# rkhosrowshahi/MO-VAE

Hardware: AMD Instinct MI355X
Metric: training images/sec (higher is better)
Workload: dtype f32

## Files before the change

### mo-vae_amd/csrc/conv_igemm.hip

```cpp
#include <cstring>
#include <cstdio>
#include "common.h"
#include <stdlib.h>

namespace {

constexpr int BK = 16;

struct Geom {
    int Nimg;
    int Hi, Wi, Cr;
    int Ho, Wo, Nn;
    int KH, KW, stride, pad;
    int wrow, wlen, wstride, woff;
};

struct Epilogue {
    const float* bias;
    int act;
    float slope;
};

struct ActMul {
    const float* y;
// ... 834 lines not shown
    RSide none{};
    if (!g_defer.pending || g_defer.st != st || g_bench_main_only) return none;
    if (g_defer.bytes > (pair ? defer_max_bytes_pair() : defer_max_bytes())) {
        (void)defer_flush();
        return none;
    }
    g_defer.pending = false;
    ++g_defer_stats[1];
    return g_defer.r;
}

inline RSide defer_take_3d(hipStream_t st, dim3* g, int* gz) {
    *gz = (int)g->z;
    RSide none{};
    if (!g_defer.pending || g_defer.st != st || g_bench_main_only) return none;
    const long layers = ((long)g_defer.r.nblk + (long)g->x * g->y - 1) / ((long)g->x * g->y);
    if ((long)g->z + layers > 65535) return none;
    if (g_defer.bytes > defer_max_bytes()) {
        (void)defer_flush();
        return none;
    }
    g->z += (unsigned)layers;
    return defer_take(st, false);
}

inline int launch_reduce_groups(const float* slab, const RGroups& rg, int G, long n1, long n2, int S, int N, const float* bias, int act,
                                float slope, int accumulate, hipStream_t st, ActMul am = ActMul{nullptr, 0, 0.f, 0, 0, nullptr},
                                bool deferrable = false) {
    if (g_bench_main_only) return MOVAE_OK;
    const long total = n1 + n2;
    uintptr_t al = reinterpret_cast<uintptr_t>(slab) | (uintptr_t)(rg.slab_gs * 4);
    for (int i = 0; i < G; ++i) al |= reinterpret_cast<uintptr_t>(rg.out[i]) | reinterpret_cast<uintptr_t>(rg.out2[i]);
    const bool al16 = (al & 15) == 0;
    RSide r{slab, rg, total, n1, S, N, accumulate, 0, 0, 0};
    if (S >= 64 && total % 4 == 0 && n1 % 4 == 0 && total <= (1L << 20) && al16) {
        r.kind = 0, r.nbx = (int)ceil_div(total, 16);
    } else if (S >= 8 && total >= reduce_vec_min() && total % 4 == 0 && n1 % 4 == 0 && al16) {
        r.kind = 1, r.nbx = (int)ceil_div(total / 4, 256);
    } else if (S >= 8 && total <= (1L << 20)) {
        r.kind = 2, r.nbx = (int)ceil_div(total, 16);
    } else {
        long gq = (total + 255) / 256;
        if (gq > 4096) gq = 4096;
        r.kind = 3, r.nbx = (int)gq;
    }
    r.nblk = r.nbx * G;
    static const char* const kind_name[4] = {"splitk_reduce_wide", "splitk_reduce_vec", "splitk_reduce", "splitk_reduce_flat"};
    note_reduce(kind_name[r.kind]);
    if (deferrable && g_defer.armed && !bias && act == MOVAE_ACT_NONE && !am.y && !am.res &&
        (size_t)total * S * G * sizeof(float) <= (defer_max_bytes() > defer_max_bytes_pair() ? defer_max_bytes() : defer_max_bytes_pair())) {
        if (int rc = defer_flush()) return rc;
        g_defer.r = r, g_defer.st = st, g_defer.pending = true, g_defer.bytes = (size_t)total * S * G * sizeof(float);
        ++g_defer.serial;
        ++g_defer_stats[0];
        return MOVAE_OK;
    }
    return reduce_launch(r, bias, act, slope, am, st);
}

inline int launch_reduce(const float* slab, float* out, long n1, int S, int N, const float* bias, int act, float slope,
                         int accumulate, hipStream_t st, float* out2 = nullptr, long n2 = 0, ActMul am = ActMul{nullptr, 0, 0.f, 0, 0, nullptr}) {
    if (!out2) n2 = 0;
    RGroups rg{};
    rg.out[0] = out, rg.out2[0] = out2, rg.slab_gs = 0;
    return launch_reduce_groups(slab, rg, 1, n1, n2, S, N, bias, act, slope, accumulate, st, am);
}

inline bool reduce_stats_shape_ok(const void* slab, const void* out, const void* part, const void* bias, long M, int N) {
    return N % 4 == 0 && N <= 1024 && 256 % (N / 4) == 0 && M <= 0x7fffffffL &&
           ((reinterpret_cast<uintptr_t>(slab) | reinterpret_cast<uintptr_t>(out) | reinterpret_cast<uintptr_t>(part)) & 15) == 0 &&
           (!bias || (reinterpret_cast<uintptr_t>(bias) & 15) == 0);
}

inline bool launch_reduce_stats(const float* slab, float* out, long M, int N, int S, const ClsSplit* scls, int Ho, int Wo, int stride,
                                const float* bias, hipStream_t st) {
    if (!g_fuse.stats || !reduce_stats_shape_ok(slab, out, g_fuse.stats, bias, M, N)) return false;
    const int RG = 256 / (N / 4);
    long rpb = 2L * RG;
    if ((M + rpb - 1) / rpb > 1024) rpb = ((M + 1023) / 1024 + RG - 1) / RG * RG;
    const long nblk = (M + rpb - 1) / rpb;
    float* part = fuse_stats_claim(nblk, N);
    if (!part) return false;
    ClsSplit one{{S, S, S, S}};
    note_reduce("splitk_reduce_stats");
    hipLaunchKernelGGL(splitk_reduce_stats, dim3((unsigned)nblk), dim3(256), 0, st, slab, out, (int)M, N, S, scls ? *scls : one, Ho, Wo,
                       scls ? stride : 0, bias, part, (int)rpb, BnBwd{});
    return true;
}

inline bool plan_reduce_bnbwd(long M, int N, BnBwd* bb, int* rows_per_block) {
    if (!g_fuse.bn_y || !g_fuse.bn_part || N % 4 != 0 || N > 1024 || 256 % (N / 4) != 0 || M > 0x7fffffffL || M % g_fuse.bn_groups != 0)
        return false;
    const long rpg = M / g_fuse.bn_groups;
    const int RG = 256 / (N / 4);
    long rpb = 2L * RG;
    while (rpb > RG && rpg % rpb != 0) rpb -= RG;
    if (rpg % rpb != 0) return false;
    while (rpg / rpb * g_fuse.bn_groups > 2048 && rpg % (rpb * 2) == 0) rpb *= 2;
    float* part = fuse_bn_claim(rpg / rpb, N);
    if (!part || ((reinterpret_cast<uintptr_t>(part) | reinterpret_cast<uintptr_t>(g_fuse.bn_y) | reinterpret_cast<uintptr_t>(g_fuse.bn_scale) |
                   reinterpret_cast<uintptr_t>(g_fuse.bn_shift)) & 15) != 0) {
        g_fuse.bn_ppg = 0;
        return false;
    }
    *bb = BnBwd{g_fuse.bn_y, g_fuse.bn_scale, g_fuse.bn_shift, g_fuse.bn_slope, part, (int)rpg, (int)(rpg / rpb)};
    *rows_per_block = (int)rpb;
    return true;
}

inline void launch_reduce_bnbwd(const float* slab, float* out, long M, int N, int S, const ClsSplit* scls, int Ho, int Wo, int stride,
                                const BnBwd& bb, int rows_per_block, hipStream_t st) {
    ClsSplit one{{S, S, S, S}};
    note_reduce("splitk_reduce_stats");
    hipLaunchKernelGGL(splitk_reduce_stats, dim3((unsigned)((M + rows_per_block - 1) / rows_per_block)), dim3(256), 0, st, slab, out, (int)M,
                       N, S, scls ? *scls : one, Ho, Wo, scls ? stride : 0, (const float*)nullptr, (float*)nullptr, rows_per_block, bb);
}

enum { FORM_FWD = 0, FORM_BWD = 1, FORM_WGRAD = 2 };
inline int choose_split(int form, int tile_area, int bk, long tiles, int nk, size_t per_slab_bytes, size_t ws_bytes, bool have_ws) {
    if (!have_ws || nk < 2) return 1;
    long smax = nk < 256 ? nk : 256;
    while (smax > 1 && per_slab_bytes * (size_t)smax > ws_bytes) --smax;
    if (g_force_split > 0) return (int)(g_force_split < smax ? g_force_split : smax);
    const bool big = tile_area >= 128 * 128;
    const double form_tk = form == FORM_FWD ? 1.0 : (form == FORM_BWD ? 1.25 : 0.9);
    const double tk = form_tk * (tile_area / 4096.0) * (big ? 0.83 : 1.0) * (bk / 32.0);
    const double out_mb = (double)per_slab_bytes * 1e-6;
    int best = 1;
    double best_t = 0.0;
    for (long S = 1; S <= smax; ++S) {
        const long kps = (nk + S - 1) / S;
        if ((nk + kps - 1) / kps != S) continue;
        const long blocks = tiles * S;
        const long rounds = (blocks + 511) / 512;
        const double share = blocks <= 256 ? 1.0 : 1.6;
        double t = rounds * (2.0 + kps * tk * share);
        if (S > 1) t += 2.5 + S * out_mb * 0.87;
        if (S == 1 || t < best_t * 0.97) {
            best = (int)S;
            best_t = t;
        }
    }
    return best;
}

inline bool pair_collecting();
template <class Plan>
inline void pair_stash(const Plan& p);
inline int pair_flush(hipStream_t st);
#include "igemm_v2.h"
#include "conv_thin.h"
#include "linear_small.h"
#include "kgemm.h"
#include "pair.h"
namespace kg {
inline bool g_force_kgemm_on() { return g_force_kgemm > 0; }
}

inline bool is_linear(const Geom& g) {
    return g.KH == 1 && g.KW == 1 && g.Hi == 1 && g.Wi == 1 && g.Ho == 1 && g.Wo == 1 && g.stride == 1 && g.pad == 0 && g.wlen == 0;
}

inline bool aligned16(const void* p) { return (reinterpret_cast<uintptr_t>(p) & 15) == 0; }

inline long big_tile_min() {
    static const long v = env_long("MOVAE_BIG_TILE_MIN", 256);
    return g_big_tile_min > 0 ? g_big_tile_min : v;
}

template <int BM, int BN>
int launch_fwd_t(const float* X, const float* W, float* Y, const Geom& g, const Epilogue& ep, int M, int K, bool vec,
                 void* ws, size_t ws_bytes, hipStream_t st) {
    const int gx = ceil_div(M, BM), gy = ceil_div(g.Nn, BN);
    const int nk = ceil_div(K, BK);
    const long tiles = (long)gx * gy;
    int S = choose_split(FORM_FWD, BM * BN, BK, tiles, nk, (size_t)M * g.Nn * sizeof(float), ws_bytes, ws != nullptr);
    const int per_split = ceil_div(nk, S);
    S = ceil_div(nk, per_split);
    float* slab = S > 1 ? static_cast<float*>(ws) : nullptr;
    dim3 grid(gx, gy, S);
    if (vec)
        hipLaunchKernelGGL((igemm_fwd<BM, BN, true>), grid, dim3(256), 0, st, X, W, Y, g, ep, M, K, per_split, slab);
    else
        hipLaunchKernelGGL((igemm_fwd<BM, BN, false>), grid, dim3(256), 0, st, X, W, Y, g, ep, M, K, per_split, slab);
    MOVAE_CHECK_LAUNCH("igemm_fwd");
    if (S > 1) {
        const long total = (long)M * g.Nn;
        if (int rc = launch_reduce(slab, Y, total, S, g.Nn, ep.bias, ep.act, ep.slope, 0, st)) return rc;
    }
    return MOVAE_OK;
}

inline bool tap_window(const Geom& g, Geom* out) {
    static const bool enabled = !getenv("MOVAE_NO_TAPWIN");
    if (!enabled || g.Ho != 1 || g.Wo != 1 || g.pad >= g.KH || g.pad >= g.KW) return false;
    const int nkh = g.KH - g.pad < g.Hi ? g.KH - g.pad : g.Hi, nkw = g.KW - g.pad < g.Wi ? g.KW - g.pad : g.Wi;
    if (nkh < 1 || nkw < 1 || nkh * nkw == g.KH * g.KW) return false;
    *out = g;
    out->KH = nkh, out->KW = nkw, out->pad = 0;
    out->wrow = g.KH * g.KW * g.Cr;
    out->wlen = nkw * g.Cr, out->wstride = g.KW * g.Cr, out->woff = (g.pad * g.KW + g.pad) * g.Cr;
    return true;
}

int launch_fwd(const float* X, const float* W, float* Y, const Geom& g_in, const Epilogue& ep, void* ws, size_t ws_bytes,
               hipStream_t st) {
    Geom g = g_in;
    {
        const long Kfull = (long)g.KH * g.KW * g.Cr;
        Geom gw;
        if (g.Cr % 4 == 0 && aligned16(X) && aligned16(W) && !is_linear(g) && !thin::thin_in_ok(g) && g.Nn > 4 && Kfull <= 0x7fffffffL &&
            tap_window(g, &gw))
            g = gw;
    }
    const long Ml = (long)g.Nimg * g.Ho * g.Wo;
    const long Kl = (long)g.KH * g.KW * g.Cr;
    if (Ml <= 0 || g.Nn <= 0 || Kl <= 0 || Ml > 0x7fffffffL) {
        movae_set_error("conv fwd-form: bad shape M=%ld N=%d K=%ld", Ml, g.Nn, Kl);
        return MOVAE_EINVAL;
    }
    const int M = (int)Ml, K = (int)Kl;
    if (is_linear(g) && lin::linear_small_ok(Ml, g.Nn, Kl) && aligned16(X) && aligned16(W)) {
        MOVAE_NO_NORM("linear (fwd)");
        float* ys[1] = {Y};
        return (g_last_kernel = "linear_small_k<NT>",
                lin::launch_linear_small<0>(X, W, ys, nullptr, 1, 0, ep.bias, M, g.Nn, K, ep.act, ep.slope, 0, st));
    }
    if (thin::thin_in_ok(g)) {
        MOVAE_NO_NORM("thin-channel input conv");
        return thin::launch_thin_in<false>(X, W, Y, g, ep, st);
    }
    if (g.Nn <= 4) {
        bool handled = false;
        if (int rc = thin::launch_thin_out_tile<false>(X, W, Y, g, ep, st, &handled)) return rc;
        if (handled) return MOVAE_OK;
    }
    if (thin::thin_out_ok(g, X)) {
        MOVAE_NO_NORM("thin-channel output conv");
        return thin::launch_thin_out_fwd(X, W, Y, g, ep, st);
    }
    const bool span_ok = v2::buf_span_ok((128L / ((long)g.Ho * g.Wo) + 2) * g.Hi * g.Wi * g.Cr) &&
                         v2::buf_span_ok((long)g.Nn * (g.wlen ? g.wrow : Kl) + g.woff);
    if (g_force_kgemm >= 0) {
        bool handled = false;
        if (int rc = kg::launch_kfwd(X, W, Y, g, ep, M, K, st, &handled)) return rc;
        if (handled) return MOVAE_OK;
    }
    if (g.Cr % 4 == 0 && aligned16(X) && aligned16(W) && span_ok) {
        if (g.Nn <= 32) return (g_last_kernel = "igemm2_fwd<128,32>", v2::launch_fwd2<128, 32>(X, W, Y, g, ep, M, K, ws, ws_bytes, st));
        if (g.Nn >= 128 && (Ml / 128) * (g.Nn / 128) >= big_tile_min()) return (g_last_kernel = g_movae_compute_bf16 ? "igemm2_fwd<128,128,true>" : "igemm2_fwd<128,128>", v2::launch_fwd2<128, 128>(X, W, Y, g, ep, M, K, ws, ws_bytes, st));
        if (Ml >= 128 * 512) return (g_last_kernel = "igemm2_fwd<128,64>", v2::launch_fwd2<128, 64>(X, W, Y, g, ep, M, K, ws, ws_bytes, st));
        return (g_last_kernel = "igemm2_fwd<64,64>", v2::launch_fwd2<64, 64>(X, W, Y, g, ep, M, K, ws, ws_bytes, st));
    }
    MOVAE_NO_NORM("generic conv (fwd form)");
    const bool vec = (g.Cr % BK == 0) && aligned16(X) && aligned16(W);
    if (g.Nn <= 32) return (g_last_kernel = vec ? "igemm_fwd<128,32,true>" : "igemm_fwd<128,32,false>", launch_fwd_t<128, 32>(X, W, Y, g, ep, M, K, vec, ws, ws_bytes, st));
    if (Ml >= 128 * 512) return (g_last_kernel = vec ? "igemm_fwd<128,64,true>" : "igemm_fwd<128,64,false>", launch_fwd_t<128, 64>(X, W, Y, g, ep, M, K, vec, ws, ws_bytes, st));
    return (g_last_kernel = vec ? "igemm_fwd<64,64,true>" : "igemm_fwd<64,64,false>", launch_fwd_t<64, 64>(X, W, Y, g, ep, M, K, vec, ws, ws_bytes, st));
}

template <int BM, int BN>
int launch_bwd_t(const float* X, const float* W, float* Y, const Geom& g, const Epilogue& ep, bool vec, void* ws,
                 size_t ws_bytes, hipStream_t st) {
    const int s = g.stride;
    const long Mmax = (long)g.Nimg * ceil_div(g.Ho, s) * ceil_div(g.Wo, s);
    const int gx = ceil_div(Mmax, BM), gy = ceil_div(g.Nn, BN);
    const int nk_max = ceil_div((long)ceil_div(g.KH, s) * ceil_div(g.KW, s) * g.Cr, BK);
    const long total = (long)g.Nimg * g.Ho * g.Wo * g.Nn;
    int S = choose_split(FORM_BWD, BM * BN, BK, (long)gx * gy * s * s, nk_max, (size_t)total * sizeof(float), ws_bytes, ws != nullptr);
    const int per_split = ceil_div(nk_max, S);
    S = ceil_div(nk_max, per_split);
    float* slab = S > 1 ? static_cast<float*>(ws) : nullptr;
    dim3 grid(gx, gy, s * s * S);
    if (vec)
        hipLaunchKernelGGL((igemm_bwd<BM, BN, true>), grid, dim3(256), 0, st, X, W, Y, g, ep, S, per_split, slab, total);
    else
        hipLaunchKernelGGL((igemm_bwd<BM, BN, false>), grid, dim3(256), 0, st, X, W, Y, g, ep, S, per_split, slab, total);
    MOVAE_CHECK_LAUNCH("igemm_bwd");
    if (S > 1) {
        if (int rc = launch_reduce(slab, Y, total, S, g.Nn, ep.bias, ep.act, ep.slope, 0, st)) return rc;
    }
    return MOVAE_OK;
}

int launch_bwd(const float* X, const float* W, float* Y, const Geom& g, const Epilogue& ep, void* ws, size_t ws_bytes,
               hipStream_t st) {
    const long Ml = (long)g.Nimg * g.Ho * g.Wo;
    if (Ml <= 0 || g.Nn <= 0 || g.Cr <= 0 || Ml > 0x7fffffffL) {
        movae_set_error("conv bwd-form: bad shape M=%ld N=%d Cr=%d", Ml, g.Nn, g.Cr);
        return MOVAE_EINVAL;
    }
    const long Mc = Ml / (g.stride * g.stride);
    if (is_linear(g) && lin::linear_small_ok(Ml, g.Nn, g.Cr) && g.Nn % 4 == 0 && aligned16(X) && aligned16(W)) {
        MOVAE_NO_NORM("linear (bwd form)");
        float* ys[1] = {Y};
        if (g_stash.collect) {
            g_stash.put(lin::make_prob<1>(X, nullptr, W, nullptr, ys, nullptr, 1, 1, 0, ep.bias, nullptr, (int)Ml, g.Nn, g.Cr, ep.act, ep.slope, 0));
            g_last_kernel = "linear_small_k<NN>";
            return MOVAE_OK;
        }
        return (g_last_kernel = "linear_small_k<NN>",
                lin::launch_linear_small<1>(X, W, ys, nullptr, 1, 0, ep.bias, (int)Ml, g.Nn, g.Cr, ep.act, ep.slope, 0, st));
    }
    if (thin::thin_in_ok(g)) {
        MOVAE_NO_NORM("thin-channel input (bwd form)");
        return thin::launch_thin_in<true>(X, W, Y, g, ep, st);
    }
    if (g.Nn <= 4) {
        bool handled = false;
        if (int rc = thin::launch_thin_out_tile<true>(X, W, Y, g, ep, st, &handled)) return rc;
        if (handled) return MOVAE_OK;
    }
    const long hwc_min = (long)(g.Ho / g.stride > 0 ? g.Ho / g.stride : 1) * (g.Wo / g.stride > 0 ? g.Wo / g.stride : 1);
    const bool span_ok = v2::buf_span_ok((128L / hwc_min + 2) * g.Hi * g.Wi * g.Cr) && v2::buf_span_ok((long)g.Cr * g.KH * g.KW * g.Nn);
    if (g_force_kgemm >= 0) {
        bool handled = false;
        if (int rc = kg::launch_kbwd(X, W, Y, g, ep, st, &handled)) return rc;
        if (handled) return MOVAE_OK;
    }
    if (g.Cr % 4 == 0 && g.Nn % 4 == 0 && g.stride <= 2 && aligned16(X) && aligned16(W) && aligned16(Y) && span_ok) {
        if (g.Nn <= 32) return (g_last_kernel = "igemm2_bwd<128,32>", v2::launch_bwd2<128, 32>(X, W, Y, g, ep, ws, ws_bytes, st));
        if (g.Nn >= 128 && (Mc / 128) * (g.Nn / 128) * g.stride * g.stride >= big_tile_min())
            return (g_last_kernel = g_movae_compute_bf16 ? "igemm2_bwd<128,128,true>" : "igemm2_bwd<128,128>", v2::launch_bwd2<128, 128>(X, W, Y, g, ep, ws, ws_bytes, st));
        if (Mc >= 128 * 512) return (g_last_kernel = "igemm2_bwd<128,64>", v2::launch_bwd2<128, 64>(X, W, Y, g, ep, ws, ws_bytes, st));
        return (g_last_kernel = "igemm2_bwd<64,64>", v2::launch_bwd2<64, 64>(X, W, Y, g, ep, ws, ws_bytes, st));
    }
    MOVAE_NO_NORM("generic conv (bwd form)");
    const bool vec = (g.Cr % BK == 0) && (g.Nn % 4 == 0) && aligned16(X) && aligned16(W);
    if (g.Nn <= 32) return (g_last_kernel = vec ? "igemm_bwd<128,32,true>" : "igemm_bwd<128,32,false>", launch_bwd_t<128, 32>(X, W, Y, g, ep, vec, ws, ws_bytes, st));
    if (Mc >= 128 * 512) return (g_last_kernel = vec ? "igemm_bwd<128,64,true>" : "igemm_bwd<128,64,false>", launch_bwd_t<128, 64>(X, W, Y, g, ep, vec, ws, ws_bytes, st));
    return (g_last_kernel = vec ? "igemm_bwd<64,64,true>" : "igemm_bwd<64,64,false>", launch_bwd_t<64, 64>(X, W, Y, g, ep, vec, ws, ws_bytes, st));
}

template <int BM, int BN>
int launch_wgrad_t(const float* S, const float* Bg, float* dW, const WGeom& g, int K, int vec, int accumulate, void* ws,
                   size_t ws_bytes, hipStream_t st) {
    const int M = g.Cs, N = g.KH * g.KW * g.Cb;
    const int gx = ceil_div(M, BM), gy = ceil_div(N, BN);
    const long tiles = (long)gx * gy;
    int Sp = choose_split(FORM_WGRAD, BM * BN, BK, tiles, ceil_div(K, BK), (size_t)M * N * sizeof(float), ws_bytes, ws != nullptr);
    int kchunk = ceil_div(ceil_div(K, Sp), BK) * BK;
    Sp = ceil_div(K, kchunk);
    const bool slab = Sp > 1 || accumulate;
    if (slab && (!ws || (size_t)M * N * sizeof(float) * Sp > ws_bytes)) {
        movae_set_error("wgrad: workspace too small (%zu bytes) for %d splits of %dx%d", ws_bytes, Sp, M, N);
        return MOVAE_EINVAL;
    }
    float* out = slab ? static_cast<float*>(ws) : dW;
    dim3 grid(gx, gy, Sp);
    const bool va = (vec & 1) != 0, vb = (vec & 2) != 0;
    if (va && vb)
        hipLaunchKernelGGL((igemm_wgrad<BM, BN, true, true>), grid, dim3(256), 0, st, S, Bg, out, g, K, kchunk, slab ? 1 : 0);
    else if (va)
        hipLaunchKernelGGL((igemm_wgrad<BM, BN, true, false>), grid, dim3(256), 0, st, S, Bg, out, g, K, kchunk, slab ? 1 : 0);
    else if (vb)
        hipLaunchKernelGGL((igemm_wgrad<BM, BN, false, true>), grid, dim3(256), 0, st, S, Bg, out, g, K, kchunk, slab ? 1 : 0);
    else
        hipLaunchKernelGGL((igemm_wgrad<BM, BN, false, false>), grid, dim3(256), 0, st, S, Bg, out, g, K, kchunk, slab ? 1 : 0);
    MOVAE_CHECK_LAUNCH("igemm_wgrad");
    if (slab) {
        const long total = (long)M * N;
        if (int rc = launch_reduce(out, dW, total, Sp, N, nullptr, 0, 0.f, accumulate, st)) return rc;
    }
    return MOVAE_OK;
}

int launch_wgrad1(const float* S, const float* Bg, float* dW, const WGeom& g, int accumulate, void* ws, size_t ws_bytes,
                  hipStream_t st) {
    const long Kl = (long)g.Nimg * g.Hs * g.Ws;
    const int vec = ((g.Cs % 4 == 0 && aligned16(S)) ? 1 : 0) | ((g.Cb % 4 == 0 && aligned16(Bg)) ? 2 : 0);
    const int N = g.KH * g.KW * g.Cb;
    if (thin::thin_wgrad_ok(g) && ws) return thin::launch_thin_wgrad(S, Bg, dW, g, (int)Kl, accumulate, ws, ws_bytes, st);
    static const char* const wgrad_name[2][4] = {
        {"igemm_wgrad<128,32,false,false>", "igemm_wgrad<128,32,true,false>", "igemm_wgrad<128,32,false,true>", "igemm_wgrad<128,32,true,true>"},
        {"igemm_wgrad<64,64,false,false>", "igemm_wgrad<64,64,true,false>", "igemm_wgrad<64,64,false,true>", "igemm_wgrad<64,64,true,true>"}};
    if (N <= 32) return (g_last_kernel = wgrad_name[0][vec], launch_wgrad_t<128, 32>(S, Bg, dW, g, (int)Kl, vec, accumulate, ws, ws_bytes, st));
    return (g_last_kernel = wgrad_name[1][vec], launch_wgrad_t<64, 64>(S, Bg, dW, g, (int)Kl, vec, accumulate, ws, ws_bytes, st));
}

int launch_wgrad(const float* S, const float* Bg, float* const* dW, int G, long s_gs, long b_gs, const WGeom& g, int accumulate,
                 void* ws, size_t ws_bytes, hipStream_t st, float* const* colsum_S = nullptr, bool* colsum_done = nullptr) {
    const long Kl = (long)g.Nimg * g.Hs * g.Ws;
    if (Kl <= 0 || Kl > 0x7fffffffL || g.Cs <= 0 || g.Cb <= 0) {
        movae_set_error("wgrad: bad shape K=%ld Cs=%d Cb=%d", Kl, g.Cs, g.Cb);
        return MOVAE_EINVAL;
    }
    if (colsum_done) *colsum_done = false;
    if (g.KH == 1 && g.KW == 1 && g.Hs == 1 && g.Ws == 1 && g.Hb == 1 && g.Wb == 1 && b_gs == 0 &&
        lin::linear_small_ok(g.Cs, g.Cb, (Kl + 3) / 4 * 4) && !g_bench_main_only) {
        MOVAE_NO_NORM("linear (wgrad)");
        if (colsum_done) *colsum_done = colsum_S != nullptr;
        if (g_stash.kind == PairStash::LINEAR) {
            g_stash.kind = PairStash::NONE, g_stash.paired = true;
            const lin::LinProb wp = lin::make_prob<2>(S, nullptr, Bg, nullptr, dW, colsum_S, G, 1, s_gs, nullptr, nullptr, g.Cs, g.Cb, (int)Kl, 0,
                                                      0.f, accumulate);
            g_last_kernel = "linear_bwd_k<false>";
            return lin::launch_linear_bwd<false>(g_stash.lin, wp, st);
        }
        return (g_last_kernel = "linear_small_k<TN>",
                lin::launch_linear_small<2>(S, Bg, dW, colsum_S, G, s_gs, nullptr, g.Cs, g.Cb, (int)Kl, 0, 0.f, accumulate, st));
    }
    const bool vec = g.Cs % 4 == 0 && g.Cb % 4 == 0 && aligned16(S) && aligned16(Bg) && s_gs % 4 == 0 && b_gs % 4 == 0 &&
                     v2::buf_span_ok(Kl * g.Cs) && v2::buf_span_ok((long)g.Nimg * g.Hb * g.Wb * g.Cb);
    const int N = g.KH * g.KW * g.Cb;
    if (g_force_kgemm >= 0 && !colsum_S && !thin::thin_wgrad_ok(g)) {
        bool handled = false;
        if (int rc = kg::launch_kwgrad(S, Bg, dW, G, s_gs, b_gs, g, (int)Kl, accumulate, ws, ws_bytes, st, &handled)) return rc;
        if (handled) return MOVAE_OK;
    }
    if (vec && !(thin::thin_wgrad_ok(g) && ws)) {
        float* const* cs = nullptr;
        if (colsum_S && !(g_fuse.nrm.scale && g_fuse.nrm_side == 1)) {
            cs = colsum_S;
            for (int i = 0; i < G; ++i)
                if (!colsum_S[i]) cs = nullptr;
        }
        if (colsum_done) *colsum_done = cs != nullptr;
        if (N <= 32) return (g_last_kernel = "igemm2_wgrad<128,32>", launch_wgrad2<128, 32>(S, Bg, dW, G, s_gs, b_gs, g, (int)Kl, accumulate, ws, ws_bytes, st, cs));
        if (g.Cs <= 32 && N >= 128) return (g_last_kernel = "igemm2_wgrad<32,128>", launch_wgrad2<32, 128>(S, Bg, dW, G, s_gs, b_gs, g, (int)Kl, accumulate, ws, ws_bytes, st, cs));
        if (g.Cs >= 128 && (long)(g.Cs / 128) * (N / 128) * (Kl / 512) * G >= big_tile_min())
            return (g_last_kernel = g_movae_compute_bf16 ? "igemm2_wgrad<128,128,true>" : "igemm2_wgrad<128,128>", launch_wgrad2<128, 128>(S, Bg, dW, G, s_gs, b_gs, g, (int)Kl, accumulate, ws, ws_bytes, st, cs));
        static const bool wide64 = !getenv("MOVAE_NO_WGRAD_64x128");
        if (wide64 && g.Cs > 32 && g.Cs <= 64 && N >= 256 && (long)(N / 128) * (Kl / 512) * G >= big_tile_min())
            return (g_last_kernel = "igemm2_wgrad<64,128>", launch_wgrad2<64, 128>(S, Bg, dW, G, s_gs, b_gs, g, (int)Kl, accumulate, ws, ws_bytes, st, cs));
        return (g_last_kernel = "igemm2_wgrad<64,64>", launch_wgrad2<64, 64>(S, Bg, dW, G, s_gs, b_gs, g, (int)Kl, accumulate, ws, ws_bytes, st, cs));
    }
    if (thin::thin_wgrad_ok(g) && ws)
        return thin::launch_thin_wgrad_grouped(S, Bg, dW, G, s_gs, b_gs, g, (int)Kl, accumulate, ws, ws_bytes, st, colsum_S, colsum_done);
    MOVAE_NO_NORM("generic wgrad");
    for (int i = 0; i < G; ++i)
        if (int rc = launch_wgrad1(S + i * s_gs, Bg + i * b_gs, dW[i], g, accumulate, ws, ws_bytes, st)) return rc;
    return MOVAE_OK;
}

int check_conv_shape(const char* who, int n, int hi, int wi, int ci, int ho, int wo, int co, int kh, int kw, int stride,
                     int pad, bool transposed) {
    if (n <= 0 || hi <= 0 || wi <= 0 || ci <= 0 || ho <= 0 || wo <= 0 || co <= 0 || kh <= 0 || kw <= 0 || stride <= 0 ||
        pad < 0) {
        movae_set_error("%s: non-positive dimension", who);
        return MOVAE_EINVAL;
    }
    if (!transposed) {
        if ((hi + 2 * pad - kh) / stride + 1 != ho || (wi + 2 * pad - kw) / stride + 1 != wo) {
            movae_set_error("%s: output %dx%d inconsistent with input %dx%d k%dx%d s%d p%d", who, ho, wo, hi, wi, kh, kw,
                            stride, pad);
            return MOVAE_EINVAL;
        }
    } else {
        const int op_h = ho - ((hi - 1) * stride - 2 * pad + kh), op_w = wo - ((wi - 1) * stride - 2 * pad + kw);
        if (op_h < 0 || op_h >= stride || op_w < 0 || op_w >= stride) {
            movae_set_error("%s: transposed output %dx%d inconsistent with input %dx%d k%dx%d s%d p%d", who, ho, wo, hi, wi,
                            kh, kw, stride, pad);
            return MOVAE_EINVAL;
        }
    }
    return MOVAE_OK;
}

}

int g_movae_compute_bf16 = 0;

struct FuseScope {
    movae_fuse_t* f;
    bool fwd;
    explicit FuseScope(movae_fuse_t* fuse, int nrm_side) : f(fuse), fwd(nrm_side == 0) {
        g_fuse = FuseCtx();
        if (!f) return;
        f->stats_parts = 0;
        if (f->in_scale && f->in_shift) g_fuse.nrm = Norm{f->in_scale, f->in_shift, f->in_slope}, g_fuse.nrm_side = nrm_side;
        if (f->stats && f->stats_cap > 0) g_fuse.stats = f->stats, g_fuse.stats_cap = f->stats_cap;
        if (fwd) {
            f->ep_act_done = 0;
            if (f->ep_res && (reinterpret_cast<uintptr_t>(f->ep_res) & 15) == 0)
                g_fuse.am = ActMul{nullptr, 0, 0.f, 0, 0, f->ep_res}, g_fuse.am_groups = 1;
        }
    }
    ~FuseScope() {
        if (f) f->stats_parts = g_fuse.stats_parts;
        if (f && fwd) f->ep_act_done = g_fuse.am_done ? 1 : 0;
        g_fuse = FuseCtx();
    }
};

struct DgradFuseScope {
    movae_fuse_t* f;
    DgradFuseScope(movae_fuse_t* fuse, int groups) : f(fuse) {
        g_fuse = FuseCtx();
        if (!f) return;
        f->bn_ppg = 0;
        f->ep_act_done = 0;
        const bool want_act = f->ep_act_y && f->ep_act != MOVAE_ACT_NONE;
        if ((want_act || f->ep_res) && groups >= 1 &&
            ((reinterpret_cast<uintptr_t>(f->ep_act_y) | reinterpret_cast<uintptr_t>(f->ep_res)) & 15) == 0)
            g_fuse.am = ActMul{want_act ? f->ep_act_y : nullptr, f->ep_act, f->ep_slope, 0, 0, f->ep_res}, g_fuse.am_groups = groups,
            g_fuse.am_done = false;
        if (f->bn_y && f->bn_scale && f->bn_shift && f->bn_part && f->bn_cap > 0 && groups >= 1) {
            g_fuse.bn_y = f->bn_y, g_fuse.bn_scale = f->bn_scale, g_fuse.bn_shift = f->bn_shift, g_fuse.bn_slope = f->bn_slope;
            g_fuse.bn_part = f->bn_part, g_fuse.bn_cap = f->bn_cap, g_fuse.bn_groups = groups;
        }
    }
    ~DgradFuseScope() {
        if (f) f->bn_ppg = g_fuse.bn_ppg, f->ep_act_done = g_fuse.am_done ? 1 : 0;
        g_fuse.bn_y = nullptr, g_fuse.bn_part = nullptr, g_fuse.bn_ppg = 0, g_fuse.bn_groups = 1;
        g_fuse.am.y = nullptr, g_fuse.am.res = nullptr, g_fuse.am_groups = 1, g_fuse.am_done = false;
    }
};
#define MOVAE_CHECK_FUSE(f, c)                                                                                                   \
    MOVAE_CHECK_ARG(!(f) || !(f)->in_scale ||                                                                                    \
                        ((f)->in_shift && (c) % 4 == 0 && ((reinterpret_cast<uintptr_t>((f)->in_scale) | reinterpret_cast<uintptr_t>((f)->in_shift)) & 15) == 0), \
                    "fused input transform: needs scale AND shift, 16-byte aligned, channels %% 4 == 0")

static int conv_fwd(bool transposed, const float* x, const float* w, const float* bias, float* y, int n, int hi, int wi, int ci, int ho,
                    int wo, int co, int kh, int kw, int stride, int pad, int act, float slope, void* ws, size_t ws_bytes,
                    movae_stream_t stream, movae_fuse_t* fuse) {
    const char* who = transposed ? "movae_convT2d_fwd" : "movae_conv2d_fwd";
    MOVAE_WS_SCRATCH(ws, ws_bytes);
    MOVAE_CHECK_ARG(x && w && y, "%s: null pointer", who);
    if (int rc = check_conv_shape(who, n, hi, wi, ci, ho, wo, co, kh, kw, stride, pad, transposed)) return rc;
    MOVAE_CHECK_FUSE(fuse, ci);
    FuseScope scope(fuse, 0);
    Geom g{n, hi, wi, ci, ho, wo, co, kh, kw, stride, pad};
    return transposed ? launch_bwd(x, w, y, g, Epilogue{bias, act, slope}, ws, ws_bytes, (hipStream_t)stream)
                      : launch_fwd(x, w, y, g, Epilogue{bias, act, slope}, ws, ws_bytes, (hipStream_t)stream);
}

static int conv_dgrad(bool transposed, const float* dy, const float* w, float* dx, int n, int hi, int wi, int ci, int ho, int wo, int co,
                      int kh, int kw, int stride, int pad, void* ws, size_t ws_bytes, movae_stream_t stream, movae_fuse_t* fuse, int groups) {
    const char* who = transposed ? "movae_convT2d_dgrad" : "movae_conv2d_dgrad";
    DgradFuseScope scope(fuse, groups);
    MOVAE_WS_SCRATCH(ws, ws_bytes);
    MOVAE_CHECK_ARG(dy && w && dx, "%s: null pointer", who);
    if (int rc = check_conv_shape(who, n, hi, wi, ci, ho, wo, co, kh, kw, stride, pad, transposed)) return rc;
    Geom g{n, ho, wo, co, hi, wi, ci, kh, kw, stride, pad};
    return transposed ? launch_fwd(dy, w, dx, g, Epilogue{nullptr, MOVAE_ACT_NONE, 0.f}, ws, ws_bytes, (hipStream_t)stream)
                      : launch_bwd(dy, w, dx, g, Epilogue{nullptr, MOVAE_ACT_NONE, 0.f}, ws, ws_bytes, (hipStream_t)stream);
}

static int conv_wgrad_grouped(bool transposed, int groups, const float* dy, const float* x, float* const* dw, float* const* dbias, int n,
                              int hi, int wi, int ci, int ho, int wo, int co, int kh, int kw, int stride, int pad, int accumulate, void* ws,
                              size_t ws_bytes, movae_stream_t stream, const movae_fuse_t* fuse) {
    const char* who = transposed ? "movae_convT2d_wgrad" : "movae_conv2d_wgrad";
    DeferArmScope defer_scope;
    MOVAE_CHECK_FUSE(fuse, ci);
    FuseScope scope(const_cast<movae_fuse_t*>(fuse), transposed ? 1 : 2);
    void* ws_full = ws;
    const size_t ws_full_bytes = ws_bytes;
    MOVAE_WS_SCRATCH(ws, ws_bytes);
    MOVAE_CHECK_ARG(dy && x && dw && groups >= 1 && groups <= 8, "%s: null pointer / bad group count", who);
    for (int i = 0; i < groups; ++i) MOVAE_CHECK_ARG(dw[i], "%s: null dw", who);
    if (int rc = check_conv_shape(who, n, hi, wi, ci, ho, wo, co, kh, kw, stride, pad, transposed)) return rc;
    const long dy_gs = (long)n * ho * wo * co;
    bool bias_done = false;
    const int rc = transposed ? launch_wgrad(x, dy, dw, groups, 0, dy_gs, WGeom{n, hi, wi, ci, ho, wo, co, kh, kw, stride, pad}, accumulate, ws,
                                             ws_bytes, (hipStream_t)stream)
                              : launch_wgrad(dy, x, dw, groups, dy_gs, 0, WGeom{n, ho, wo, co, hi, wi, ci, kh, kw, stride, pad}, accumulate, ws,
                                             ws_bytes, (hipStream_t)stream, dbias, &bias_done);
    if (rc) return rc;
    if (dbias && !bias_done && !g_bench_main_only && g_defer.pending && g_defer.serial != defer_scope.serial)
        if (int rc2 = defer_flush()) return rc2;
    if (dbias && !bias_done && !g_bench_main_only)
        for (int i = 0; i < groups; ++i)
            if (dbias[i])
                if (int rc2 = movae_colsum(dy + i * dy_gs, dbias[i], n * ho * wo, co, accumulate, ws_full, ws_full_bytes, stream)) return rc2;
    return MOVAE_OK;
}

static int conv_dgrad_wgrad_grouped(bool transposed, int groups, const float* dy, const float* w, const float* x, float* dx, float* const* dw,
                                    float* const* dbias, int n, int hi, int wi, int ci, int ho, int wo, int co, int kh, int kw, int stride,
                                    int pad, int accumulate, void* ws, size_t ws_bytes, movae_stream_t stream, const movae_fuse_t* fuse) {
    static const bool enabled = !getenv("MOVAE_NO_PAIR");
    MOVAE_CHECK_ARG(dx && w, "%s: null pointer", transposed ? "movae_convT2d_dgrad_wgrad" : "movae_conv2d_dgrad_wgrad");
    g_stash.clear();
    g_stash.collect = enabled;
    int rc = conv_dgrad(transposed, dy, w, dx, groups * n, hi, wi, ci, ho, wo, co, kh, kw, stride, pad, ws, ws_bytes, stream,
                        const_cast<movae_fuse_t*>(fuse), groups);
    g_stash.collect = false;
    const char* dgrad_kernel = g_last_kernel;
    if (rc) {
        g_stash.clear();
        return rc;
    }
    size_t used = (g_stash.ws_used + 255) / 256 * 256;
    if (g_stash.kind == PairStash::TILE && (!ws || used + (32u << 20) > ws_bytes)) {
        if ((rc = g_stash.flush((hipStream_t)stream))) return rc;
        used = 0;
    }
    rc = conv_wgrad_grouped(transposed, groups, dy, x, dw, dbias, n, hi, wi, ci, ho, wo, co, kh, kw, stride, pad, accumulate,
                            ws ? static_cast<char*>(ws) + used : nullptr, ws_bytes - used, stream, fuse);
    const int rc2 = g_stash.flush((hipStream_t)stream);
    if (!rc) rc = rc2;
    if (!g_stash.paired) {
        static thread_local char both[128];
        snprintf(both, sizeof(both), "%s + %s", dgrad_kernel, g_last_kernel);
        g_last_kernel = both;
    }
    return rc;
}

extern "C" {

const char* movae_bench_last_kernel(void) { return g_last_kernel; }

const char* movae_bench_last_reduce(void) {
    static char out[sizeof(g_last_reduce)];
    memcpy(out, g_last_reduce, g_last_reduce_len + 1);
    g_last_reduce[0] = 0, g_last_reduce_len = 0;
    return out;
}

int movae_reduce_defer(int on) {
    const int prev = g_defer.armed ? 1 : 0;
    g_defer.armed = on != 0;
    return prev;
}

int movae_reduce_flush(void) { return defer_flush(); }

long long movae_reduce_defer_max_bytes(long long bytes) {
    const long long prev = (long long)g_defer_max_bytes;
    if (bytes >= 0) g_defer_max_bytes = g_defer_max_bytes_pair = (size_t)bytes;
    return prev;
}

int movae_reduce_defer_stats(long long* out3, int reset) {
    if (out3)
        for (int i = 0; i < 3; ++i) out3[i] = g_defer_stats[i];
    if (reset) g_defer_stats[0] = g_defer_stats[1] = g_defer_stats[2] = 0;
    return g_defer.pending ? 1 : 0;
}

int movae_bench_force_split(int s) {
    const int prev = g_force_split;
    g_force_split = s > 0 ? s : 0;
    return prev;
}

int movae_set_compute_dtype(int dtype) {
    const int prev = g_movae_compute_bf16 ? MOVAE_DTYPE_BF16 : MOVAE_DTYPE_F32;
    g_movae_compute_bf16 = dtype == MOVAE_DTYPE_BF16 ? 1 : 0;
    return prev;
}

int movae_bench_force_kgemm(int mode) {
    const int prev = g_force_kgemm;
    g_force_kgemm = mode > 0 ? 1 : (mode < 0 ? -1 : 0);
    return prev;
}

int movae_bench_big_tile_min(int n) {
    const int prev = g_big_tile_min;
    g_big_tile_min = n > 0 ? n : 0;
    return prev;
}

int movae_bench_main_kernel_only(int on) {
    const int prev = g_bench_main_only ? 1 : 0;
    g_bench_main_only = on != 0;
    return prev;
}

int movae_conv2d_fwd_f(const float* x, const float* w, const float* bias, float* y, int n, int hi, int wi, int ci, int ho,
                       int wo, int co, int kh, int kw, int stride, int pad, int act, float slope, void* ws, size_t ws_bytes,
                       movae_stream_t stream, movae_fuse_t* fuse) {
    return conv_fwd(false, x, w, bias, y, n, hi, wi, ci, ho, wo, co, kh, kw, stride, pad, act, slope, ws, ws_bytes, stream, fuse);
}

int movae_conv2d_fwd(const float* x, const float* w, const float* bias, float* y, int n, int hi, int wi, int ci, int ho,
                     int wo, int co, int kh, int kw, int stride, int pad, int act, float slope, void* ws, size_t ws_bytes,
                     movae_stream_t stream) {
    return conv_fwd(false, x, w, bias, y, n, hi, wi, ci, ho, wo, co, kh, kw, stride, pad, act, slope, ws, ws_bytes, stream, nullptr);
}

int movae_conv2d_dgrad(const float* dy, const float* w, float* dx, int n, int hi, int wi, int ci, int ho, int wo, int co,
                       int kh, int kw, int stride, int pad, void* ws, size_t ws_bytes, movae_stream_t stream) {
    return conv_dgrad(false, dy, w, dx, n, hi, wi, ci, ho, wo, co, kh, kw, stride, pad, ws, ws_bytes, stream, nullptr, 1);
// ... 172 lines not shown
```

Before: 331,600.

## Add sub-pixel class-decomposed MFMA kernel for stride-2 3x3 transposed conv forward

Adds a dedicated kernel for the forward pass of stride-2, pad-1, 3x3 transposed convolutions with 32 in and 32 out channels on 8- or 16-wide inputs. It splits the output into four parity classes, each using only its 1, 2, 2 or 4 contributing taps, and runs them on fp32 MFMA from LDS-resident weights and input tiles. Input normalisation, bias, activation and batch-norm statistics are fused into the kernel. This avoids the zero-tap waste and generic tiling of the igemm2 backward path for these decoder layers, at the cost of a large LDS footprint and a path that only applies to this narrow shape set.

```diff
diff --git a/mo-vae_amd/csrc/conv_igemm.hip b/mo-vae_amd/csrc/conv_igemm.hip
--- a/mo-vae_amd/csrc/conv_igemm.hip
+++ b/mo-vae_amd/csrc/conv_igemm.hip
@@ -1010,6 +1010,7 @@
 #include "conv_thin.h"
 #include "linear_small.h"
 #include "kgemm.h"
+#include "convt_img.h"
 #include "pair.h"
 namespace kg {
 inline bool g_force_kgemm_on() { return g_force_kgemm > 0; }
@@ -1142,7 +1143,7 @@
 }
 
 int launch_bwd(const float* X, const float* W, float* Y, const Geom& g, const Epilogue& ep, void* ws, size_t ws_bytes,
-               hipStream_t st) {
+               hipStream_t st, bool convt_fwd = false) {
     const long Ml = (long)g.Nimg * g.Ho * g.Wo;
     if (Ml <= 0 || g.Nn <= 0 || g.Cr <= 0 || Ml > 0x7fffffffL) {
         movae_set_error("conv bwd-form: bad shape M=%ld N=%d Cr=%d", Ml, g.Nn, g.Cr);
@@ -1176,6 +1177,7 @@
         if (int rc = kg::launch_kbwd(X, W, Y, g, ep, st, &handled)) return rc;
         if (handled) return MOVAE_OK;
     }
+    if (convt_fwd && img::img_ok(X, W, Y, g, ep)) return img::launch_img(X, W, Y, g, ep, st);
     if (g.Cr % 4 == 0 && g.Nn % 4 == 0 && g.stride <= 2 && aligned16(X) && aligned16(W) && aligned16(Y) && span_ok) {
         if (g.Nn <= 32) return (g_last_kernel = "igemm2_bwd<128,32>", v2::launch_bwd2<128, 32>(X, W, Y, g, ep, ws, ws_bytes, st));
         if (g.Nn >= 128 && (Mc / 128) * (g.Nn / 128) * g.stride * g.stride >= big_tile_min())
@@ -1379,7 +1381,7 @@
     MOVAE_CHECK_FUSE(fuse, ci);
     FuseScope scope(fuse, 0);
     Geom g{n, hi, wi, ci, ho, wo, co, kh, kw, stride, pad};
-    return transposed ? launch_bwd(x, w, y, g, Epilogue{bias, act, slope}, ws, ws_bytes, (hipStream_t)stream)
+    return transposed ? launch_bwd(x, w, y, g, Epilogue{bias, act, slope}, ws, ws_bytes, (hipStream_t)stream, true)
                       : launch_fwd(x, w, y, g, Epilogue{bias, act, slope}, ws, ws_bytes, (hipStream_t)stream);
 }
 
diff --git a/mo-vae_amd/csrc/convt_img.h b/mo-vae_amd/csrc/convt_img.h
--- /dev/null
+++ b/mo-vae_amd/csrc/convt_img.h
@@ -0,0 +1,232 @@
+#pragma once
+
+namespace img {
+
+constexpr int CI = 32;
+constexpr int GPB = 4;
+constexpr int LDX = 57;
+constexpr int OUT_G = 4096;
+constexpr int WROW = 288;
+constexpr int XIT = 7;
+constexpr int MAIN = CI * WROW + GPB * CI * LDX;
+constexpr int LDS_BYTES = MAIN * 4;
+static_assert(MAIN >= 4 * 128 * 32, "the four classes' 128 x 32 tiles fit the operand memory");
+
+struct ImgArgs {
+    const float* X;
+    const float* W;
+    float* Y;
+    const float* bias;
+    int act;
+    float slope;
+    Norm nrm;
+    float* stats;
+    int groups;
+    int hi;
+    FastDiv fd_gpi;
+};
+
+__device__ constexpr int NTAP[4] = {1, 2, 2, 4};
+__device__ constexpr int TAP[4][4] = {{4, 0, 0, 0}, {3, 5, 0, 0}, {1, 7, 0, 0}, {0, 2, 6, 8}};
+__device__ constexpr int SHIFT[4][4] = {{0, 0, 0, 0}, {1, 0, 0, 0}, {2, 0, 0, 0}, {3, 2, 1, 0}};
+
+template <int CA, int CB, int PW>
+__device__ __forceinline__ void img_mma(const float* __restrict__ xa, const float* __restrict__ wb, f32x16 (&acc)[4]) {
+    constexpr int SA = NTAP[CA] * 16, STEPS = SA + NTAP[CB] * 16;
+    constexpr int D = 4;
+    float a[D], b[D];
+    auto fetch = [&](int st, int s) {
+        const int c = st < SA ? CA : CB, u = st < SA ? st : st - SA;
+        const int i = u >> 4, j = u & 15;
+        const int sh = SHIFT[c][i];
+        a[s] = xa[j * LDX + (sh & 1) + (sh >> 1) * PW];
+        b[s] = wb[j * WROW + TAP[c][i] * 32];
+    };
+#pragma unroll
+    for (int st = 0; st < D - 1; ++st) fetch(st, st);
+#pragma unroll
+    for (int st = 0; st < STEPS; ++st) {
+        const int s = st % D;
+        if (st + D - 1 < STEPS) fetch(st + D - 1, (st + D - 1) % D);
+        __builtin_amdgcn_sched_barrier(0);
+        if (st < SA) acc[CA] = __builtin_amdgcn_mfma_f32_32x32x2f32(a[s], b[s], acc[CA], 0, 0, 0);
+        else acc[CB] = __builtin_amdgcn_mfma_f32_32x32x2f32(a[s], b[s], acc[CB], 0, 0, 0);
+        __builtin_amdgcn_sched_barrier(0);
+    }
+}
+
+template <int CA, int CB, int LW, bool ACT>
+__device__ __forceinline__ void img_store(float* __restrict__ yg, f32x16 (&acc)[4], float bias, int act, float slope, int half) {
+    constexpr int wi = 1 << LW;
+    yg += half * 2 * 4 * 32;
+#pragma unroll
+    for (int k = 0; k < 2; ++k) {
+        const int c = k ? CB : CA;
+        const int dh = c >> 1, dw = c & 1;
+#pragma unroll
+        for (int r = 0; r < 16; ++r) {
+            const int p = acc_row(r, 0);
+            const int pr = p >> LW, pc = p & (wi - 1);
+            float v = acc[c][r] + bias;
+            if (ACT) v = v > 0.f ? v : (act == MOVAE_ACT_RELU ? 0.f : v * slope);
+            acc[c][r] = v;
+            yg[((2 * pr + dh) * 2 * wi + 2 * pc + dw) * 32] = v;
+        }
+    }
+}
+
+template <int LW>
+__global__ __launch_bounds__(256) void igemm2_bwd_img(ImgArgs a) {
+    constexpr int Q = CI / 4;
+    extern __shared__ __attribute__((aligned(16))) float lds[];
+    float* const wsm = lds;
+    float* const xsm = lds + CI * WROW;
+    const int t = threadIdx.x;
+    const int g0 = blockIdx.x * GPB;
+    constexpr int wi = 1 << LW, R = 32 >> LW, pw = wi + 1;
+    constexpr int gitems = (R + 1) * pw * Q;
+    const int hi = a.hi;
+    const int q = t & (Q - 1);
+
+    constexpr int WIT = CI * WROW / 4 / 256;
+    f32x4 wv[WIT];
+#pragma unroll
+    for (int i = 0; i < WIT; ++i) wv[i] = reinterpret_cast<const f32x4*>(a.W)[i * 256 + t];
+    f32x4 xv[XIT];
+    int xoff[XIT];
+    bool xin[XIT];
+#pragma unroll
+    for (int i = 0; i < XIT; ++i) {
+        const int idx = t + i * 256;
+        const int g = idx / gitems;
+        const int pos = (idx - g * gitems) / Q;
+        const int r = pos / pw, c = pos - r * pw;
+        const int gi = g0 + g;
+        const int im = fdiv(gi, a.fd_gpi);
+        const int row = (gi - im * (hi >> (5 - LW))) * R + r;
+        const bool in_block = g < GPB;
+        const bool valid = in_block && gi < a.groups && row < hi && c < wi;
+        xoff[i] = in_block ? (g * CI + 4 * q) * LDX + pos : -1;
+        xin[i] = valid;
+        xv[i] = f32x4{0.f, 0.f, 0.f, 0.f};
+        if (valid) xv[i] = *reinterpret_cast<const f32x4*>(a.X + (((size_t)im * hi + row) * wi + c) * CI + 4 * q);
+    }
+    if (a.nrm.scale) {
+        const f32x4 sc = *reinterpret_cast<const f32x4*>(a.nrm.scale + 4 * q), sh = *reinterpret_cast<const f32x4*>(a.nrm.shift + 4 * q);
+#pragma unroll
+        for (int i = 0; i < XIT; ++i) xv[i] = norm_apply_if(xin[i], xv[i], sc, sh, a.nrm.slope);
+    }
+#pragma unroll
+    for (int i = 0; i < XIT; ++i) {
+        if (xoff[i] >= 0) {
+            float* d = xsm + xoff[i];
+            d[0] = xv[i][0], d[LDX] = xv[i][1], d[2 * LDX] = xv[i][2], d[3 * LDX] = xv[i][3];
+        }
+    }
+#pragma unroll
+    for (int i = 0; i < WIT; ++i) reinterpret_cast<f32x4*>(wsm)[i * 256 + t] = wv[i];
+    __syncthreads();
+
+    const int g = t >> 6, lane = t & 63, half = lane >> 5, l31 = lane & 31;
+    const bool live = g0 + g < a.groups;
+    f32x16 acc[4];
+#pragma unroll
+    for (int c = 0; c < 4; ++c)
+#pragma unroll
+        for (int r = 0; r < 16; ++r) acc[c][r] = 0.f;
+    if (live) {
+        const float* xa = xsm + (g * CI + half * 16) * LDX + (l31 >> LW) * pw + (l31 & (wi - 1));
+        const float* wb = wsm + half * 16 * WROW + l31;
+        float* const yg = a.Y + (size_t)(g0 + g) * OUT_G + l31;
+        const float bias = a.bias ? a.bias[l31] : 0.f;
+        const bool plain = a.act == MOVAE_ACT_NONE;
+        img_mma<0, 1, pw>(xa, wb, acc);
+        if (plain) img_store<0, 1, LW, false>(yg, acc, bias, a.act, a.slope, half);
+        else img_store<0, 1, LW, true>(yg, acc, bias, a.act, a.slope, half);
+        img_mma<2, 3, pw>(xa, wb, acc);
+        if (plain) img_store<2, 3, LW, false>(yg, acc, bias, a.act, a.slope, half);
+        else img_store<2, 3, LW, true>(yg, acc, bias, a.act, a.slope, half);
+    }
+    if (!a.stats) return;
+
+    __syncthreads();
+    float* const S = lds;
+    if (live) {
+#pragma unroll
+        for (int c = 0; c < 4; ++c)
+#pragma unroll
+            for (int r = 0; r < 16; ++r) S[(c * 128 + g * 32 + acc_row(r, half)) * 32 + l31] = acc[c][r];
+    }
+    __syncthreads();
+    const int nlive = a.groups - g0 < GPB ? a.groups - g0 : GPB;
+    const int cq = t & 7, rowi = t >> 3;
+    f32x4 s1[4], s2[4];
+#pragma unroll
+    for (int c = 0; c < 4; ++c) {
+        s1[c] = f32x4{0.f, 0.f, 0.f, 0.f}, s2[c] = s1[c];
+#pragma unroll
+        for (int u = 0; u < 4; ++u) {
+            if (u < nlive) {
+                const f32x4 v = *reinterpret_cast<const f32x4*>(S + (c * 128 + rowi + 32 * u) * 32 + cq * 4);
+                s1[c] += v;
+#pragma unroll
+                for (int j = 0; j < 4; ++j) s2[c][j] = fmaf(v[j], v[j], s2[c][j]);
+            }
+        }
+    }
+    __syncthreads();
+    float* const F = lds;
+#pragma unroll
+    for (int c = 0; c < 4; ++c) {
+        *reinterpret_cast<f32x4*>(F + ((c * 2 + 0) * 32 + rowi) * 32 + cq * 4) = s1[c];
+        *reinterpret_cast<f32x4*>(F + ((c * 2 + 1) * 32 + rowi) * 32 + cq * 4) = s2[c];
+    }
+    __syncthreads();
+    if (t < 128) {
+        const int c = t >> 5, col = t & 31;
+        float c1 = 0.f, c2 = 0.f;
+        for (int i = 0; i < 32; ++i) c1 += F[((c * 2 + 0) * 32 + i) * 32 + col], c2 += F[((c * 2 + 1) * 32 + i) * 32 + col];
+        const size_t pidx = (size_t)c * gridDim.x + blockIdx.x;
+        a.stats[(pidx * 2 + 0) * 32 + col] = c1;
+        a.stats[(pidx * 2 + 1) * 32 + col] = c2;
+    }
+}
+
+template <int LW>
+inline int launch_img_t(const ImgArgs& a, hipStream_t st) {
+    static bool lds_set = false;
+    if (!lds_set) {
+        if (hipFuncSetAttribute(reinterpret_cast<const void*>(igemm2_bwd_img<LW>), hipFuncAttributeMaxDynamicSharedMemorySize, LDS_BYTES) !=
+            hipSuccess) {
+            (void)hipGetLastError();
+            movae_set_error("igemm2_bwd_img: %d bytes of LDS refused", LDS_BYTES);
+            return MOVAE_EUNSUPPORTED;
+        }
+        lds_set = true;
+    }
+    hipLaunchKernelGGL((igemm2_bwd_img<LW>), dim3((unsigned)ceil_div(a.groups, GPB)), dim3(256), LDS_BYTES, st, a);
+    MOVAE_CHECK_LAUNCH("igemm2_bwd_img");
+    return MOVAE_OK;
+}
+
+inline bool img_ok(const float* X, const float* W, const float* Y, const Geom& g, const Epilogue& ep) {
+    const long px = (long)g.Hi * g.Wi;
+    return g.KH == 3 && g.KW == 3 && g.stride == 2 && g.pad == 1 && g.Ho == 2 * g.Hi && g.Wo == 2 * g.Wi && g.Nn == 32 && g.Cr == CI &&
+           (g.Wi == 8 || g.Wi == 16) && px % 32 == 0 && px <= 256 && kg::al16(X) && kg::al16(W) && kg::al16(Y) && kg::al16(ep.bias) &&
+           kg::al16(g_fuse.nrm.scale) && kg::al16(g_fuse.nrm.shift) && !g_movae_compute_bf16 && !g_fuse.am.y && !g_fuse.am.res && !g_fuse.bn_y &&
+           (ep.act == MOVAE_ACT_NONE || ep.act == MOVAE_ACT_LRELU || ep.act == MOVAE_ACT_RELU) && (long)g.Nimg * px / 32 <= 0x3fffffffL;
+}
+
+inline int launch_img(const float* X, const float* W, float* Y, const Geom& g, const Epilogue& ep, hipStream_t st) {
+    if (int rc = defer_flush()) return rc;
+    ImgArgs a{};
+    a.X = X, a.W = W, a.Y = Y, a.bias = ep.bias, a.act = ep.act, a.slope = ep.slope, a.nrm = g_fuse.nrm;
+    a.groups = (int)((long)g.Nimg * g.Hi * g.Wi / 32);
+    a.hi = g.Hi;
+    a.fd_gpi = fastdiv_make(g.Hi * g.Wi / 32);
+    if (g_fuse.stats && ep.act == MOVAE_ACT_NONE) a.stats = fuse_stats_claim(4L * ceil_div(a.groups, GPB), 32);
+    g_last_kernel = "igemm2_bwd_img<32>";
+    return g.Wi == 8 ? launch_img_t<3>(a, st) : launch_img_t<4>(a, st);
+}
+
+}
```

Result: no change. 337,900, median of 6 (+1.9%).
